# danieleschmidt/grid-fed-rl-gym

Measured on AMD Instinct MI355X. Metric: env steps/sec (batched feeders), higher is better.
Workload: dtype f64

## Files before the change

### grid_fed_rl_gym_amd/csrc/env_device.h

```cpp
#pragma once
#include <hip/hip_runtime.h>
#include <math.h>

#include "gs_internal.h"
#include "fastmath.h"

#ifndef ROW
#define ROW(r) S[(size_t)(r) * GS_LANES]
#endif

template <typename X>
__device__ __forceinline__ X cld(const X* p, int i) {
  return ((const GS_CONST X*)p)[i];
}

__device__ __forceinline__ double hour_of_day(double time_s) {
  return gs_fmod_pos(gs_div_by(time_s, 3600.0, 1.0 / 3600.0), 24.0, 1.0 / 24.0);
}

struct U4 { uint32_t a, b, c, d; };

__device__ __forceinline__ U4 philox(uint32_t c0, uint32_t c1, uint32_t c2, uint32_t c3, uint32_t k0, uint32_t k1) {
#pragma unroll
  for (int r = 0; r < 10; ++r) {
// ... 166 lines not shown
      ROW(R.SOC + q) = soc;
      ROW(R.BATP + q) = -(e * 3600.0 / dt);
    }
  }
#pragma unroll
  for (int g = 0; g < 8; ++g) { if (g >= T.n_gens) break; ROW(R.CURT + g) = (a_g[g] + 1.0) / 2.0; }
  for (int g = 8; g < T.n_gens; ++g) ROW(R.CURT + g) = (act[T.n_bats + g] + 1.0) / 2.0;
  ROW(R.TIME) = t_old + dt;
  ROW(R.STEP) = k_old + 1.0;
}

__device__ __forceinline__ double load_power_z(const GsTables& T, int l, double z, double prof) {
  return fmax(0.0, cld(T.load_base, l) * (prof * (1.0 + 0.1 * z)) * 1.0);
}
template <typename TablePtr>
__device__ __forceinline__ double daily_profile_from(TablePtr table, double time_s) {
  const double hour = hour_of_day(time_s);
  const int hi = (int)hour;
  const double frac = hour - (double)hi;
  return table[hi] * (1.0 - frac) + table[(hi + 1) % 24] * frac;
}
__device__ __forceinline__ double daily_profile(double time_s) { return daily_profile_from(kDailyProfile, time_s); }

__device__ __forceinline__ void bus_injection(const GsTables& T, const GsRows& R, const GsEnvCfg& E, GsLaneRows S, int i) {
  double ls = 0.0, gs = 0.0;
  for (int p = cld(T.bl_ptr, i); p < cld(T.bl_ptr, i + 1); ++p) ls += ROW(R.LOADP + cld(T.bl_idx, p));
  for (int p = cld(T.bg_ptr, i); p < cld(T.bg_ptr, i + 1); ++p) {
    const int g = cld(T.bg_idx, p);
    gs += ROW(R.GENP + g) * ROW(R.CURT + g);
  }
  for (int p = cld(T.bb_ptr, i); p < cld(T.bb_ptr, i + 1); ++p) {
    const double bp = ROW(R.BATP + cld(T.bb_idx, p));
    if (bp > 0.0) gs += bp; else if (bp < 0.0) ls += fabs(bp);
  }
  ROW(R.P + i) = (0.0 - gs_div_by(ls, E.power_base, E.inv_power_base)) + gs_div_by(gs, E.power_base, E.inv_power_base);
  ROW(R.Q + i) = 0.0;
}

__device__ __forceinline__ void env_reset_lane_scalars(const GsTables& T, const GsRows& R, const GsEnvCfg& E, GsLaneRows S,
                                                       uint64_t inst, uint64_t seed) {
  ROW(R.SEEDLO) = (double)(uint32_t)seed;
  ROW(R.SEEDHI) = (double)(uint32_t)(seed >> 32);
  ROW(R.TIME) = 0.0; ROW(R.STEP) = 0.0; ROW(R.VIOL) = 0.0; ROW(R.TOTLOSS) = 0.0; ROW(R.EPREW) = 0.0;
  ROW(R.FREQ) = 60.0;
  ROW(R.IRR) = 0.0; ROW(R.WIND) = 5.0; ROW(R.TEMP) = 25.0; ROW(R.CLOUD) = 0.3;
  for (int q = 0; q < T.n_bats; ++q) { ROW(R.SOC + q) = 0.5; ROW(R.BATP + q) = 0.0; }
// ... 25 lines not shown
```

### grid_fed_rl_gym_amd/csrc/gridstep_abi.hip

```cpp
#include <hip/hip_runtime.h>

#include <dlfcn.h>

#include <algorithm>
#include <cmath>
#include <cstdarg>
#include <cstdio>
#include <cstdlib>
#include <cstring>
#include <string>
#include <vector>

#include "../../include/gridstep.h"
#include "gs_internal.h"
#include "kernels.h"
#include "topology.h"
#include "mesh_schedule.h"
#include "plan.h"
#include "policy.h"

namespace {

thread_local std::string g_last_error;

// ... 33 lines not shown
  a.CommCuDevice = (int (*)(gs_ncclComm_t, int*))dlsym(lib, "ncclCommCuDevice");
  a.GetVersion = (int (*)(int*))dlsym(lib, "ncclGetVersion");
  a.GetErrorString = (const char* (*)(int))dlsym(lib, "ncclGetErrorString");
  if (!a.GetUniqueId || !a.CommInitRank || !a.AllGather || !a.CommDestroy) { why = "librccl lacks a required symbol"; return false; }
  g_rccl = a;
  return true;
}

struct TimedLaunch { int kid; hipEvent_t a, b; };
constexpr size_t GS_CHECKS_MAX_EVENTS = 4096;

}

struct gs_handle : GsPlan {
  int device = 0;
  hipStream_t stream = nullptr;
  gs_config cfg{};
  HostTopology topo;
  GsTables T{};
  struct gs_checks* fused = nullptr;
  bool forked = false;
  hipStream_t stream2 = nullptr; hipEvent_t ev_fork = nullptr, ev_join = nullptr, ev_peer = nullptr, ev_peer2 = nullptr;
  bool rows_stale = false; const double* last_obs = nullptr;
  unsigned long long* d_stamps = nullptr;
  bool was_reset = false;
  std::vector<void*> allocs;
  char* arena = nullptr; size_t arena_left = 0;
  double* slab = nullptr;
  double* d_in = nullptr; size_t in_doubles = 0;
  double* d_out = nullptr; size_t out_doubles = 0;
  double* d_obs2[2] = {nullptr, nullptr}; int obs_cur = 0;
  hipStream_t comm_stream = nullptr; hipEvent_t ev_step = nullptr, ev_gather[2] = {nullptr, nullptr}; bool gather_pending[2] = {false, false};
  std::vector<const double*> bound_obs;
  float* d_obs32 = nullptr;
  hipEvent_t ev_scalars = nullptr;
  double* d_actions = nullptr; int n_action_batches = 0;
  struct Rollout {
    int T_cap = 0, T = 0, term_cap = 0; uint64_t calls = 0;
    double* obs_seq = nullptr; double* act = nullptr; double* rew = nullptr; uint8_t* done = nullptr;
    int32_t* term_count = nullptr; int32_t* term_idx = nullptr; double* term_obs = nullptr;
    int32_t n_term = 0;
  } ro;
  struct Policy { bool set = false; double* blob = nullptr; double* act = nullptr; GsPolicyArgs args{}; int compute = GS_COMPUTE_F64; GsPolicyArgsF32 args32{}; int lds32 = 0; } pol;
  double* d_cst = nullptr;
  int32_t *map_obs = nullptr, *map_vm = nullptr, *map_va = nullptr, *map_flow = nullptr, *map_load = nullptr,
          *map_p = nullptr, *map_q = nullptr, *map_act = nullptr, *map_state = nullptr;
// ... 122 lines not shown
  HIPCHK(h, hipGetLastError());
  return GS_OK;
}

int launch_pack_obs(gs_handle* h, double* dst) {
  const int rc = launch_pack(h, h->map_obs, h->obs_dim, dst);
  if (rc || !h->pl) return rc;
  const size_t threads = (size_t)h->B * 2 * h->n_loads;
  hipLaunchKernelGGL(gs_k_load_columns, dim3((unsigned)((threads + 255) / 256)), dim3(256), 0, h->stream, (const double*)h->LL.pl, dst, h->B, h->obs_dim,
                     2 * h->n + 2 * h->m + 1, h->n_loads);
  HIPCHK(h, hipGetLastError());
  return GS_OK;
}

int launch_unpack(gs_handle* h, const int32_t* map, int C, const double* src, int stride = 0) {
  if (C <= 0) return GS_OK;
  LaunchTimer lt(h, GS_K_UNPACK);
  dim3 grid(h->groups, (C + 63) / 64);
  hipLaunchKernelGGL(gs_k_unpack, grid, dim3(256), 0, h->stream, map, C, h->R.total, h->slab, src, h->B, stride ? stride : C);
  HIPCHK(h, hipGetLastError());
  return GS_OK;
}

int ensure_rows(gs_handle* h) {
  if (!h->rows_stale) return GS_OK;
  h->rows_stale = false;
  return launch_unpack(h, h->map_obs, 2 * h->n + 2 * h->m, h->last_obs, h->obs_dim);
}

int pack_to_host(gs_handle* h, const int32_t* map, int C, double* host) {
  if (!host || C <= 0) return GS_OK;
  int rc = launch_pack(h, map, C, h->d_out);
  if (rc) return rc;
  HIPCHK(h, hipMemcpyAsync(host, h->d_out, (size_t)h->B * C * sizeof(double), hipMemcpyDeviceToHost, h->stream));
  HIPCHK(h, hipStreamSynchronize(h->stream));
  return GS_OK;
}

int unpack_from_host(gs_handle* h, const int32_t* map, int C, const double* host) {
  if (C <= 0) return GS_OK;
  HIPCHK(h, hipMemcpyAsync(h->d_in, host, (size_t)h->B * C * sizeof(double), hipMemcpyHostToDevice, h->stream));
  return launch_unpack(h, map, C, h->d_in);
}

int fetch_scalars(gs_handle* h, bool sync = true) {
  hipLaunchKernelGGL(gs_k_scalars, dim3(h->groups), dim3(64), 0, h->stream, h->rows_f, (int)SF_COUNT, h->rows_i,
                     (int)SI_COUNT, h->rows_u, (int)SU_COUNT, h->R.total, h->slab, h->hd_f, h->hd_i, h->hd_u, h->Bp, h->hd_v4, (int)SU_VF0);
// ... 31 lines not shown
  return GS_OK;
}

GsFusedChecks fused_checks_args(gs_handle* h);

int step_kernels(gs_handle* h, const double* d_actions, double* obs_out = nullptr, const GsRolloutStep* rs = nullptr) {
  { LaunchTimer lt(h, GS_K_SOLVE);
    dim3 grid(h->groups), block(64 * h->W);
    if (!obs_out) {
      const int next = h->obs_cur ^ 1;
      if (h->gather_pending[next]) {
        HIPCHK(h, hipStreamWaitEvent(h->stream, h->ev_gather[next], 0));
        if (h->split_ok) HIPCHK(h, hipStreamWaitEvent(h->stream2, h->ev_gather[next], 0));
        h->gather_pending[next] = false;
      }
      h->obs_cur = next;
      obs_out = h->d_obs2[next];
    }
    GsPackArgs pa{h->map_obs, h->d_cst, obs_out, h->obs_dim, (int)std::max<size_t>(1, std::min<size_t>(3, (h->dyn_lds - 49152) / (64 * 65 * sizeof(double)))), 0, 0,
                  h->obs_skip0, h->obs_skip1};
    pa.pair_ok = !(h->obs_dim & 1) && !((h->obs_skip1 - h->obs_skip0) & 1) && pa.tiles_per_pass >= 2 && !GS_EXPERIMENT_ENV("GS_PACK_BY_COLUMN");
    pa.early_pass0 = 2 * h->n + 2 * h->m >= 64 * pa.tiles_per_pass;
    pa.lean = h->lean ? 1 : 0;
    if (h->lean) { h->rows_stale = true; h->last_obs = obs_out; }
    const GsFusedChecks fc = fused_checks_args(h);
    const GsRolloutStep rsv = rs ? *rs : GsRolloutStep{};
    if (h->second_gen()) {
      const int per_group = 64 / h->f2().iw, n_wg = h->groups * per_group;
      const dim3 b2(64 * h->f2().nw);
      const bool split = h->split_ok && !h->timing;
      const int n_first = split ? (h->groups / 2) * per_group : n_wg;
      if (split && !h->forked) {
        HIPCHK(h, hipEventRecord(h->ev_fork, h->stream));
        HIPCHK(h, hipStreamWaitEvent(h->stream2, h->ev_fork, 0));
        h->forked = true;
      }
      GsF2Tables f2a = h->F2, f2b = h->F2;
      f2a.wg_offset = 0; f2b.wg_offset = n_first;
      auto launch = [&](auto k, auto... pz) -> int {
        if (!k) return fail(h, GS_E_STATE, "%s: no such step kernel", h->f2().name);
        hipLaunchKernelGGL(k, dim3(n_first), b2, h->F2.lds_bytes, h->stream, h->T, f2a, h->R, h->SC, h->EC, h->slab, h->B, d_actions, h->total_load, pa, fc, rsv, pz...);
        if (n_first < n_wg)
          hipLaunchKernelGGL(k, dim3(n_wg - n_first), b2, h->F2.lds_bytes, h->stream2, h->T, f2b, h->R, h->SC, h->EC, h->slab, h->B, d_actions, h->total_load, pa, fc, rsv, pz...);
        return GS_OK;
      };
      const GsStepKernels& k = gs_step_kernels[(int)h->step];
      const double *pz = h->LP.pz, *pl = h->LL.pl;
// ... 436 lines not shown
  if (mask) HIPCHK(h, hipMemcpyAsync(h->d_pzmask, mask, (size_t)h->B, hipMemcpyHostToDevice, h->stream));
  int rc = launch_line_params(h, mask ? h->d_pzmask : nullptr);
  if (rc) return rc;
  HIPCHK(h, hipStreamSynchronize(h->stream));
  return GS_OK;
}

int gs_get_line_impedances(const gs_handle* h, double* r, double* x) {
  if (!h) return fail(nullptr, GS_E_INVALID, "handle is NULL");
  if (!h->pz) return fail(const_cast<gs_handle*>(h), GS_E_STATE, "gs_get_line_impedances: the handle has no per-instance line impedances");
  if (r) std::copy(h->inst_r.begin(), h->inst_r.end(), r);
  if (x) std::copy(h->inst_x.begin(), h->inst_x.end(), x);
  return GS_OK;
}

int gs_set_load_powers(gs_handle* h, const double* base, const uint8_t* mask) {
  if (!h) return fail(nullptr, GS_E_INVALID, "handle is NULL");
  if (!h->pl) return fail(h, GS_E_STATE, "gs_set_load_powers: the handle was created without per-instance load powers "
                                         "(gs_topology::load_base_inst)");
  if (!base) return fail(h, GS_E_INVALID, "gs_set_load_powers: base is [B][n_loads]");
  const std::string why = gs_check_load_powers(h->n_loads, h->B, base, mask);
  if (!why.empty()) return fail(h, GS_E_INVALID, "%s", why.c_str());
  GS_ENTER(h);
  const size_t nl = (size_t)h->n_loads;
  for (int b = 0; b < h->B; ++b) {
    if (mask && !mask[b]) continue;
    std::copy(base + b * nl, base + (b + 1) * nl, h->inst_load.begin() + b * nl);
  }
  HIPCHK(h, hipMemcpyAsync(const_cast<double*>(h->LL.base), h->inst_load.data(), h->inst_load.size() * sizeof(double), hipMemcpyHostToDevice, h->stream));
  if (mask) HIPCHK(h, hipMemcpyAsync(h->d_plmask, mask, (size_t)h->B, hipMemcpyHostToDevice, h->stream));
  int rc = launch_load_params(h, mask ? h->d_plmask : nullptr);
  if (rc) return rc;
  HIPCHK(h, hipStreamSynchronize(h->stream));
  return GS_OK;
}

int gs_get_load_powers(const gs_handle* h, double* base) {
  if (!h) return fail(nullptr, GS_E_INVALID, "handle is NULL");
  if (!h->pl) return fail(const_cast<gs_handle*>(h), GS_E_STATE, "gs_get_load_powers: the handle has no per-instance load powers");
  if (base) std::copy(h->inst_load.begin(), h->inst_load.end(), base);
  return GS_OK;
}

static const char* const kPzNoSolve = "gs_solve / gs_solve_device: this handle has per-instance line impedances, which the solver API does not "
                                      "support (the step, rollout and fallback entry points do)";
int gs_upload_injections(gs_handle* h, const double* P_spec, const double* Q_spec) {
  if (!h || !P_spec) return fail(h, GS_E_INVALID, "handle / P_spec is NULL");
  if (h->pz) return fail(h, GS_E_STATE, "%s", kPzNoSolve);
  GS_ENTER(h);
  int rc = unpack_from_host(h, h->map_p, h->n, P_spec);
  if (rc) return rc;
  if (Q_spec) {
    HIPCHK(h, hipStreamSynchronize(h->stream));
    rc = unpack_from_host(h, h->map_q, h->n, Q_spec);
    if (rc) return rc;
  } else {
    hipLaunchKernelGGL(gs_k_fill_rows, dim3(h->groups), dim3(64), 0, h->stream, h->R.Q.base, 2, h->n, h->R.total, h->slab, 0.0);
    HIPCHK(h, hipGetLastError());
  }
  HIPCHK(h, hipStreamSynchronize(h->stream));
  return GS_OK;
}

int gs_solve_device(gs_handle* h) {
  if (!h) return fail(nullptr, GS_E_INVALID, "handle is NULL");
  if (h->pz) return fail(h, GS_E_STATE, "%s", kPzNoSolve);
  GS_ENTER(h);
  h->rows_stale = false;
  return launch_solve(h);
}

int gs_download_solution(gs_handle* h, const gs_solution_view* out) {
  if (!h || !out) return fail(h, GS_E_INVALID, "handle / view is NULL");
  GS_ENTER(h);
  int rc;
  if ((rc = ensure_rows(h))) return rc;
  if ((rc = pack_to_host(h, h->map_vm, h->n, out->bus_voltages))) return rc;
  if ((rc = pack_to_host(h, h->map_va, h->n, out->bus_angles))) return rc;
  if ((rc = pack_to_host(h, h->map_flow, h->m, out->line_flows))) return rc;
  if ((rc = pack_to_host(h, h->map_load, h->m, out->line_loadings))) return rc;
  if ((rc = fetch_scalars(h))) return rc;
  const int B = h->B, Bp = h->Bp;
  if (out->losses) memcpy(out->losses, h->h_f + (size_t)SF_LOSSES * Bp, B * sizeof(double));
  if (out->max_mismatch) memcpy(out->max_mismatch, h->h_f + (size_t)SF_MAXMIS * Bp, B * sizeof(double));
  if (out->iterations) memcpy(out->iterations, h->h_i + (size_t)SI_ITERS * Bp, B * sizeof(int32_t));
  if (out->status) memcpy(out->status, h->h_i + (size_t)SI_STATUS * Bp, B * sizeof(int32_t));
  if (out->converged) memcpy(out->converged, h->h_u + (size_t)SU_CONV * Bp, B);
  return GS_OK;
}

// ... 326 lines not shown
  gs_handle::Rollout& ro = h->ro;
  const size_t B = h->B, D = h->obs_dim, A = h->action_dim;
  ro.T = T; ro.n_term = -1;
  HIPCHK(h, hipMemsetAsync(ro.term_count, 0, sizeof(int32_t), h->stream));
  if (A > 0) {
    if (policy == GS_POLICY_UPLOADED) {
      HIPCHK(h, hipMemcpyAsync(ro.act, actions, (size_t)T * B * A * sizeof(double), hipMemcpyHostToDevice, h->stream));
    } else if (policy == GS_POLICY_RANDOM) {
      const long long total = (long long)T * B * ((A + 3) / 4);
      hipLaunchKernelGGL(gs_k_rollout_actions, dim3((unsigned)((total + 255) / 256)), dim3(256), 0, h->stream, ro.act, (int)T, (int)B, (int)A,
                         policy_seed, h->EC.first_instance, 0u);
      HIPCHK(h, hipGetLastError());
    }
  }
  HIPCHK(h, hipMemcpyAsync(ro.obs_seq, h->d_obs2[h->obs_cur], B * D * sizeof(double), hipMemcpyDeviceToDevice, h->stream));
  const bool fused = h->second_gen() && policy != GS_POLICY_MLP;
  for (int t = 0; t < T; ++t) {
    double* nxt = ro.obs_seq + (size_t)(t + 1) * B * D;
    if (policy == GS_POLICY_MLP && (rc = launch_policy(h, ro.obs_seq + (size_t)t * B * D, ro.act + (size_t)t * B * A, policy_seed, t))) return rc;
    GsRolloutStep rs{ro.rew, ro.done, ro.obs_seq + (size_t)t * B * D, h->map_obs, h->d_cst, ro.term_count, ro.term_idx, ro.term_obs, ro.term_cap, h->obs_dim, t, 1};
    if ((rc = step_kernels(h, ro.act + (size_t)t * B * A, nxt, fused ? &rs : nullptr))) return rc;
    if (!fused || t == T - 1) {
      if ((rc = join_streams(h))) return rc;
      GsRolloutPostArgs pa{fused ? nullptr : ro.rew, fused ? nullptr : ro.done, nxt, h->map_obs, h->d_cst, ro.term_count, ro.term_idx, ro.term_obs, ro.term_cap, h->obs_dim, t, h->B};
      hipLaunchKernelGGL(gs_k_rollout_post, dim3(h->groups), dim3(256), 0, h->stream, h->T, h->R, h->EC, h->slab, pa);
      HIPCHK(h, hipGetLastError());
      if (h->pl) {
        const size_t threads = (size_t)h->B * 2 * h->n_loads;
        hipLaunchKernelGGL(gs_k_load_columns, dim3((unsigned)((threads + 255) / 256)), dim3(256), 0, h->stream, (const double*)h->LL.pl, nxt, h->B,
                           h->obs_dim, 2 * h->n + 2 * h->m + 1, h->n_loads);
        HIPCHK(h, hipGetLastError());
      }
    }
  }
  if ((rc = join_streams(h))) return rc;
  if (h->gather_pending[h->obs_cur]) { HIPCHK(h, hipStreamWaitEvent(h->stream, h->ev_gather[h->obs_cur], 0)); h->gather_pending[h->obs_cur] = false; }
  HIPCHK(h, hipMemcpyAsync(h->d_obs2[h->obs_cur], ro.obs_seq + (size_t)T * B * D, B * D * sizeof(double), hipMemcpyDeviceToDevice, h->stream));
  if (h->rows_stale) h->last_obs = h->d_obs2[h->obs_cur];
  ro.calls += 1;
  return GS_OK;
}

static int rollout_finish(gs_handle* h) {
  gs_handle::Rollout& ro = h->ro;
  if (ro.T <= 0) return fail(h, GS_E_STATE, "no rollout has been collected on this handle");
  GS_ENTER(h);
  if (ro.n_term < 0) {
// ... 34 lines not shown
  if (ro.n_term && out->next_observations) {
    HIPCHK(h, hipMemcpyAsync(idx.data(), ro.term_idx, idx.size() * sizeof(int32_t), hipMemcpyDeviceToHost, h->stream));
    HIPCHK(h, hipMemcpyAsync(rows.data(), ro.term_obs, rows.size() * sizeof(double), hipMemcpyDeviceToHost, h->stream));
  }
  HIPCHK(h, hipStreamSynchronize(h->stream));
  if (out->next_observations)
    for (int k = 0; k < ro.n_term; ++k)
      memcpy(out->next_observations + ((size_t)idx[2 * k] * B + idx[2 * k + 1]) * D, rows.data() + (size_t)k * D, D * sizeof(double));
  if (out->n_terminal) *out->n_terminal = ro.n_term;
  return GS_OK;
}

int gs_get_state(gs_handle* h, double* state) {
  if (!h || !state) return fail(h, GS_E_INVALID, "handle / state is NULL");
  GS_ENTER(h);
  int rc = ensure_rows(h);
  if (rc) return rc;
  return pack_to_host(h, h->map_state, h->state_dim, state);
}

int gs_set_state(gs_handle* h, const double* state) {
  if (!h || !state) return fail(h, GS_E_INVALID, "handle / state is NULL");
  GS_ENTER(h);
  h->rows_stale = false;
  int rc = unpack_from_host(h, h->map_state, h->state_dim, state);
  if (rc) return rc;
  hipLaunchKernelGGL(gs_k_polar_to_rect, dim3(h->groups), dim3(64), 0, h->stream, h->T, h->R, h->slab, h->B);
  HIPCHK(h, hipGetLastError());
  if (h->comm_stream) HIPCHK(h, hipStreamSynchronize(h->comm_stream));
  h->gather_pending[0] = h->gather_pending[1] = false;
  if ((rc = launch_pack_obs(h, h->d_obs2[h->obs_cur]))) return rc;
  HIPCHK(h, hipMemcpyAsync(h->d_obs2[h->obs_cur ^ 1], h->d_obs2[h->obs_cur], (size_t)h->B * h->obs_dim * sizeof(double), hipMemcpyDeviceToDevice, h->stream));
  HIPCHK(h, hipStreamSynchronize(h->stream));
  h->was_reset = true;
  return GS_OK;
}

int gs_comm_unique_id(uint8_t id_out[128]) {
  std::string why;
  if (!load_rccl(why)) return fail(nullptr, GS_E_COMM, "%s", why.c_str());
  gs_ncclUniqueId id;
  int rc = g_rccl.GetUniqueId(&id);
  if (rc != 0) return fail(nullptr, GS_E_COMM, "ncclGetUniqueId: %s", g_rccl.GetErrorString ? g_rccl.GetErrorString(rc) : "error");
  memcpy(id_out, id.internal, 128);
  return GS_OK;
}
// ... 693 lines not shown
```

### grid_fed_rl_gym_amd/csrc/gs_internal.h

```cpp
#pragma once
#include <stdint.h>

#if defined(GS_BUILD_EXPERIMENTS)
#define GS_EXPERIMENT_ENV(name) getenv(name)
#else
#define GS_EXPERIMENT_ENV(name) ((const char*)nullptr)
#endif

#define GS_LANES 64
#define GS_ELEM(row, lane) ((((size_t)(row) >> 1) << 7) + ((size_t)(lane) << 1) + ((size_t)(row) & 1))
#define GS_MAX_WAVES 16
#define GS_ELL_K 4

#if defined(__HIP_DEVICE_COMPILE__)
#define GS_CONST __attribute__((address_space(4)))
#else
#define GS_CONST
#endif

#define GS_ARGS_IN_PLACE(Block, name)                                                                                           \
  const __attribute__((address_space(4))) char* ka_ = (const __attribute__((address_space(4))) char*)__builtin_amdgcn_kernarg_segment_ptr(); \
  asm volatile("" : "+s"(ka_));                                                                                                \
  const Block* name = (const Block*)ka_

// ... 312 lines not shown
  int32_t n_slots;
  int32_t slack;
  int32_t n_jump;
  int32_t n_levels, pos_off, n_anc_ints, wg_offset;
  int32_t off_tile, off_anc, off_z, off_env, off_red, off_atom, lds_bytes;
  int32_t off_prof, ring_zero;
  int32_t env_genp, env_curt, env_batp, env_soc;
  int32_t n_fixed, fixed_slot0;
  double fixed_val0;
  const int32_t* fixed_slot; const double* fixed_val;
  double* nrflat; int32_t nrflat_mode, pad_nrflat;
  const int32_t* mesh_items; const int32_t* mesh_rowinfo;
  int32_t off_scr, mesh_nz;
  int32_t mesh_pairs, mesh_off_p;
  const double* mesh_w; int32_t mesh_w_steps, mesh_slack;
};

struct GsRolloutPostArgs {
  double* rew; uint8_t* done;
  double* obs_next;
  const int32_t* map; const double* cst;
  int32_t* term_count; int32_t* term_idx; double* term_obs; int32_t term_cap;
  int32_t obs_dim, t, B;
};

struct GsRolloutStep {
  double* rew; uint8_t* done;
  double* obs_prev;
  const int32_t* map; const double* cst;
  int32_t* term_count; int32_t* term_idx; double* term_obs;
  int32_t term_cap, obs_dim, t, active;
};

#define GS_STAMP_BLOCKS 2048
struct GsSolveCfg {
  double tolerance, alpha;
  int32_t max_iterations, jacobian_exact;
  unsigned long long* stamps;
  int32_t stamp_wave, block_times;
};

struct GsEnvCfg {
  double timestep, v_min, v_max, f_min, f_max, safety_penalty, H, D, f0, power_base, inv_power_base;
  int32_t episode_length, stochastic_loads, weather_variation, fbs_warm_start;
  int64_t first_instance;
};
// ... 43 lines not shown
```

### grid_fed_rl_gym_amd/csrc/kernels.h

```cpp
#pragma once
#include <hip/hip_runtime.h>

#include <array>

#include "gs_internal.h"
#include "members.h"
#include "policy.h"

typedef void (*GsSolveFn)(GsTables T, GsRows R, GsSolveCfg C, double* slab, int B);
typedef void (*GsStepFn)(GsTables T, GsRows R, GsSolveCfg C, GsEnvCfg E, double* slab, int B, const double* actions, double total_load,
                         GsPackArgs PA, GsFusedChecks FC);
typedef void (*GsF2StepFn)(GsTables T, GsF2Tables F, GsRows R, GsSolveCfg C, GsEnvCfg E, double* slab, int B, const double* actions,
                           double total_load, GsPackArgs PA, GsFusedChecks FC, GsRolloutStep RS);
typedef void (*GsF2StepPzFn)(GsTables T, GsF2Tables F, GsRows R, GsSolveCfg C, GsEnvCfg E, double* slab, int B, const double* actions,
                             double total_load, GsPackArgs PA, GsFusedChecks FC, GsRolloutStep RS, const double* pz);
template <class Fn> struct GsStepFns { Fn step = nullptr, stepc = nullptr; };
struct GsSolveKernels { GsSolveFn solve; GsStepFns<GsStepFn> step; };
typedef void (*GsF2StepPzPlFn)(GsTables T, GsF2Tables F, GsRows R, GsSolveCfg C, GsEnvCfg E, double* slab, int B, const double* actions,
                               double total_load, GsPackArgs PA, GsFusedChecks FC, GsRolloutStep RS, const double* pz, const double* pl);
struct GsStepKernels { GsStepFns<GsF2StepFn> plain; GsStepFns<GsF2StepPzFn> pz, pl; GsStepFns<GsF2StepPzPlFn> pz_pl; };
extern const std::array<GsSolveKernels, (size_t)SolveMember::nr_sparse_lds + 1> gs_solve_kernels;
extern const std::array<GsStepKernels, kStepMemberCount> gs_step_kernels;

extern "C" {
__global__ void gs_k_line_params(GsLineParamArgs A);
__global__ void gs_k_load_params(GsLoadParamArgs A);
__global__ void gs_k_load_columns(const double* __restrict__ pl, double* __restrict__ out, int B, int obs_dim, int c0, int n_loads);
__global__ void gs_k_pre_nr_dmfma(GsTables T, GsRows R, GsSolveCfg C, GsEnvCfg E, double* __restrict__ slab, int B,
                                  const double* __restrict__ actions, double total_load, GsPackArgs PA, GsFusedChecks FC);
__global__ void gs_k_post_nr_dmfma(GsTables T, GsRows R, GsSolveCfg C, GsEnvCfg E, double* __restrict__ slab, int B,
                                   const double* __restrict__ actions, double total_load, GsPackArgs PA, GsFusedChecks FC);
__global__ void gs_k_postc_nr_dmfma(GsTables T, GsRows R, GsSolveCfg C, GsEnvCfg E, double* __restrict__ slab, int B,
                                    const double* __restrict__ actions, double total_load, GsPackArgs PA, GsFusedChecks FC);
__global__ void gs_k_posts_nr_dmfma(GsTables T, GsRows R, GsSolveCfg C, double* __restrict__ slab, int B);
__global__ void gs_k_nr_dense_mfma(GsDenseArgs A, double* __restrict__ slab, int B);
__global__ void gs_k_nr_dense_mfma2(GsDenseArgs A, double* __restrict__ slab, int B);
__global__ void gs_k_nr_sparse_lds(GsSparseArgs A, double* __restrict__ slab, int B);
__global__ void gs_k_env_reset(GsTables T, GsRows R, GsEnvCfg E, double* __restrict__ slab, int B,
                               const uint64_t* __restrict__ seeds, const uint8_t* __restrict__ mask);
__global__ void gs_k_polar_to_rect(GsTables T, GsRows R, double* __restrict__ slab, int B);
__global__ void gs_k_rollout_actions(double* __restrict__ act, int T, int B, int A, uint64_t seed, int64_t first_instance, uint32_t t0);
__global__ void gs_k_fill_const_columns(double* __restrict__ out, long long rows, int obs_dim, int skip0, int skip1,
                                        const int32_t* __restrict__ map, const double* __restrict__ cst);
__global__ void gs_k_policy_mlp(GsPolicyArgs P);
__global__ void gs_k_policy_mlp_f32(GsPolicyArgsF32 P);
__global__ void gs_k_rollout_post(GsTables T, GsRows R, GsEnvCfg E, double* __restrict__ slab, GsRolloutPostArgs A);
__global__ void gs_k_pack(const int32_t* __restrict__ src, const double* __restrict__ cst, int C, int rows_total,
                          const double* __restrict__ slab, double* __restrict__ out, int B);
__global__ void gs_k_unpack(const int32_t* __restrict__ dst, int C, int rows_total, double* __restrict__ slab,
                            const double* __restrict__ in, int B, int stride);
__global__ void gs_k_obs_compact(const double* __restrict__ src, double* __restrict__ dst, long long rows, int D, int skip0, int skip1, int expand);
__global__ void gs_k_obs_to_f32(const double* __restrict__ src, float* __restrict__ dst, long long n);
__global__ void gs_k_gather_lane(int row0, int count, int lane, const double* __restrict__ slab, double* __restrict__ out);
__global__ void gs_k_fill_rows(int row0, int stride, int count, int rows_total, double* __restrict__ slab, double value);
__global__ void gs_k_scalars(const int32_t* __restrict__ rf, int nf, const int32_t* __restrict__ ri, int ni,
                             const int32_t* __restrict__ ru, int nu, int rows_total, const double* __restrict__ slab,
                             double* __restrict__ of, int32_t* __restrict__ oi, uint8_t* __restrict__ ou, int Bp, uint32_t* __restrict__ ov4, int vf0);
__global__ void gs_k_checks(GsChecksCfg C, const double* __restrict__ slab, const double* __restrict__ freq_override,
                            double* __restrict__ prev, int32_t* __restrict__ state, int32_t* __restrict__ out_i,
                            double* __restrict__ out_f, uint8_t* __restrict__ bus_mask, uint8_t* __restrict__ line_mask, int B, int Bp);
__global__ void gs_k_fallback_linear(GsTables T, GsRows R, GsFallbackArgs A, double* __restrict__ slab, int B);
__global__ void gs_k_checks_reset(int32_t* __restrict__ state, const uint8_t* __restrict__ mask, int B, int Bp);
}
```

### grid_fed_rl_gym_amd/csrc/kernels_env.hip

```cpp
#include <hip/hip_runtime.h>
#include <math.h>

#include "gs_internal.h"

#define ROW(r) S[(size_t)(r) * GS_LANES]
#include "env_device.h"

extern "C" __global__ void __launch_bounds__(64)
gs_k_env_reset(GsTables T, GsRows R, GsEnvCfg E, double* __restrict__ slab, int B,
               const uint64_t* __restrict__ seeds, const uint8_t* __restrict__ mask) {
  const int lane = threadIdx.x;
  const int b = blockIdx.x * GS_LANES + lane;
  const GsLaneRows S = gs_lane_rows(slab, blockIdx.x, R.total, lane);
  if (b >= B) return;
  if (mask && !mask[b]) return;
  const uint64_t inst = (uint64_t)(E.first_instance + b);
  const uint64_t seed = seeds ? seeds[b] : next_episode_seed(lane_seed(S, R), inst);
  env_reset_lane(T, R, E, S, inst, seed);
}

extern "C" __global__ void __launch_bounds__(64)
gs_k_polar_to_rect(GsTables T, GsRows R, double* __restrict__ slab, int B) {
  const int lane = threadIdx.x;
  const int b = blockIdx.x * GS_LANES + lane;
  const GsLaneRows S = gs_lane_rows(slab, blockIdx.x, R.total, lane);
  if (b >= B) return;
  for (int i = 0; i < T.n; ++i) {
    const double vm = ROW(R.VM + i), va = ROW(R.VA + i);
    double s, c;
    sincos(va, &s, &c);
    ROW(R.E + i) = vm * c; ROW(R.F + i) = vm * s;
  }
  for (int g = 0; g < T.n_gens; ++g) ROW(R.GENP + g) = renewable_power(T, R, S, g);
}

extern "C" __global__ void __launch_bounds__(256)
gs_k_rollout_actions(double* __restrict__ act, int T, int B, int A, uint64_t seed, int64_t first_instance, uint32_t t0) {
  const int Aq = (A + 3) >> 2;
  const long long idx = (long long)blockIdx.x * blockDim.x + threadIdx.x;
  if (idx >= (long long)T * B * Aq) return;
  const int q = (int)(idx % Aq);
  const long long tb = idx / Aq;
  const int b = (int)(tb % B), t = (int)(tb / B);
  const U4 r = philox((uint32_t)(first_instance + b), t0 + (uint32_t)t, (uint32_t)q, 0x4143544Eu, (uint32_t)seed, (uint32_t)(seed >> 32));
  const uint32_t w[4] = {r.a, r.b, r.c, r.d};
  double* o = act + ((size_t)t * B + b) * A + 4 * q;
#pragma unroll
  for (int k = 0; k < 4; ++k)
    if (4 * q + k < A) o[k] = 2.0 * (((double)w[k] + 0.5) * (1.0 / 4294967296.0)) - 1.0;
}

extern "C" __global__ void __launch_bounds__(256)
gs_k_fill_const_columns(double* __restrict__ out, long long rows, int obs_dim, int skip0, int skip1,
                        const int32_t* __restrict__ map, const double* __restrict__ cst) {
  const int w = skip1 - skip0;
  const long long idx = (long long)blockIdx.x * blockDim.x + threadIdx.x;
// ... 18 lines not shown
        A.rew[(size_t)A.t * A.B + b] = rew;
        A.done[(size_t)A.t * A.B + b] = (uint8_t)d;
      }
      if (d) {
        k = atomicAdd(A.term_count, 1);
        if (k < A.term_cap) { A.term_idx[2 * k] = A.t; A.term_idx[2 * k + 1] = b; }
        else k = -1;
      }
    }
    fin[lane] = k;
  }
  __syncthreads();
  bool any = false;
  for (int q = 0; q < GS_LANES; ++q) {
    const int k = fin[q];
    any |= k != -2;
    if (k >= 0) {
      const double* row = A.obs_next + (size_t)(blockIdx.x * GS_LANES + q) * A.obs_dim;
      double* dst = A.term_obs + (size_t)k * A.obs_dim;
      for (int c = threadIdx.x; c < A.obs_dim; c += blockDim.x) dst[c] = row[c];
    }
  }
  if (!any) return;
  if (mine && fin[lane] != -2) {
    const uint64_t inst = (uint64_t)(E.first_instance + b);
    env_reset_lane_scalars(T, R, E, S, inst, next_episode_seed(lane_seed(S, R), inst));
  }
  for (int q = 0; q < GS_LANES; ++q) {
    if (fin[q] == -2) continue;
    const GsLaneRows Sq = gs_lane_rows(slab, blockIdx.x, R.total, q);
    for (int j = threadIdx.x; j < T.n + T.m; j += blockDim.x) env_reset_element(T, R, Sq, j);
  }
  asm volatile("s_waitcnt vmcnt(0) lgkmcnt(0)\n\ts_barrier" ::: "memory");
  for (int q = 0; q < GS_LANES; ++q) {
    if (fin[q] == -2) continue;
    const GsLaneRows Sq = gs_lane_rows(slab, blockIdx.x, R.total, q);
    double* row = A.obs_next + (size_t)(blockIdx.x * GS_LANES + q) * A.obs_dim;
    for (int c = threadIdx.x; c < A.obs_dim; c += blockDim.x) {
      const int s = A.map[c];
      row[c] = (s >= 0) ? Sq.lane_row((size_t)s * GS_LANES).get() : A.cst[-s - 1];
    }
  }
}
```

### grid_fed_rl_gym_amd/csrc/kernels_flow2.hip

```cpp
#include <hip/hip_runtime.h>
#include <math.h>
#include <limits.h>
#include <type_traits>
#include <utility>

#include "../../include/gridstep.h"
#include "gs_internal.h"
#include "kernels.h"
#include "members.h"

#define ROW(r) S[(size_t)(r) * GS_LANES]
#include "env_device.h"

#pragma clang fp contract(off)

extern __shared__ __attribute__((aligned(16))) char f2_lds[];

__device__ __forceinline__ void f2_sync() { asm volatile("s_waitcnt vmcnt(0) lgkmcnt(0)\n\ts_barrier" ::: "memory"); }
__device__ __forceinline__ void f2_lds_sync() { asm volatile("s_waitcnt lgkmcnt(0)\n\ts_barrier" ::: "memory"); }

#define F2_AS3 __attribute__((address_space(3)))
#define F2_P(type, off) ((type F2_AS3*)((F2_AS3 char*)f2_lds + (off)))
#define F2_VP(type, off) ((volatile type F2_AS3*)((F2_AS3 char*)f2_lds + (off)))
typedef double f2_v2 __attribute__((ext_vector_type(2)));
// ... 311 lines not shown
      if (on) { if (valid) f2_row(S, R.CURT + gi) = c; env_lds[(F.env_curt + gi) * IW + l] = c; }
    }
    if (valid && hv == 0) { ROW(R.TIME) = told + dt; ROW(R.STEP) = kold + 1.0; }
  }
  if (wave == (NW >= 2 ? 1 : 0)) {
    const GsWeather wx = weather_step(R, E, S, inst, tnew, snew, valid);
    const double elev = solar_elevation(valid ? tnew : told);
    for (int g0 = 0; g0 < ng; g0 += HV) {
      const int gi = g0 + hv; const bool on = gi < ng; const int gg = on ? gi : 0;
      const double cap = T.gen_cap[gg], p0 = T.gen_p0[gg], p1 = T.gen_p1[gg], p2 = T.gen_p2[gg];
      double pw;
      if (T.gen_kind[gg] == 0) {
        const double irr = 1000.0 * elev * (1.0 - 0.8 * wx.cloud);
        const double tf = 1.0 - 0.004 * fmax(0.0, wx.temp - 25.0);
        pw = fmin(irr * p1 * p0 * tf, cap);
      } else if (wx.wind < p0 || wx.wind > p2) pw = 0.0;
      else if (wx.wind <= p1) { const double q = (wx.wind - p0) / (p1 - p0); pw = cap * (q * q * q); }
      else pw = cap;
      if (on) { f2_row(S, R.GENP + gi) = pw; env_lds[(F.env_genp + gi) * IW + l] = pw; }
    }
  }
  if (NW < 3 || wave >= 2) {
    const double prof = E.stochastic_loads ? daily_profile_from(F2_P(const double, o_prof), tnew) : 1.0;
    for (int p = (NW < 3 ? wave : wave - 2) * HV + hv; 4 * p < nl_; p += (NW < 3 ? NW : NW - 2) * HV) {
      const int l0 = 4 * p;
      double base4[4];
#pragma unroll
      for (int k = 0; k < 4; ++k) base4[k] = PL ? 0.0 : T.load_base[min(l0 + k, nl_ - 1)];
      if constexpr (PL != 0) {
        const double2 b01 = pl_at(2 * p), b23 = pl_at(min(2 * p + 1, GS_PL_NP(nl_) - 1));
        base4[0] = b01.x; base4[1] = b01.y; base4[2] = b23.x; base4[3] = b23.y;
      }
      double z[4] = {0.0, 0.0, 0.0, 0.0};
      if (E.stochastic_loads) rng_normal_quad(seed, inst, snew, DRAW_LOAD0 + p, z);
      double lp[4];
#pragma unroll
      for (int k = 0; k < 4; ++k) {
        const double base = base4[k];
        lp[k] = E.stochastic_loads ? fmax(0.0, base * (prof * (1.0 + 0.1 * z[k])) * 1.0) : base;
        if (l0 + k < nl_) loadp_lds[(l0 + k) * IW + l] = lp[k];
      }
      if (l0 + 1 < nl_) f2_pair(S, R.LOADP + l0) = make_double2(lp[0], lp[1]); else f2_row(S, R.LOADP + l0) = lp[0];
      if (l0 + 3 < nl_) f2_pair(S, R.LOADP + l0 + 2) = make_double2(lp[2], lp[3]); else if (l0 + 2 < nl_) f2_row(S, R.LOADP + l0 + 2) = lp[2];
    }
  }
  stp.hit(F2_ST_PRO_SPARE);
  f2_lds_sync();
  stp.hit(F2_ST_PRO_SCALAR);

  double Pj[NI], IR[NI], II[NI], JR[NI], JI[NI];
#pragma unroll
  for (int j = 0; j < NI; ++j) {
    if constexpr (SOLVER == F2_NRM) { rdev[j][0] = *(const f2_i4*)&rec0[j].nl; rdev[j][1] = *(const f2_i4*)&rec0[j].g0; rdev_b1[j] = rec0[j].b1; }
    const int nl = rdev[j][0].x, l0 = rdev[j][0].y, l1 = rdev[j][0].z, ngj = rdev[j][0].w, g0 = rdev[j][1].x, g1 = rdev[j][1].y,
              nbj = rdev[j][1].z, b0 = rdev[j][1].w, b1 = rdev_b1[j];
    double ls = 0.0, gs = 0.0;
    if (nl > 0) ls += loadp_lds[l0 * IW + l];
    if (nl > 1) ls += loadp_lds[l1 * IW + l];
    if (ngj > 0) gs += env_lds[(F.env_genp + g0) * IW + l] * env_lds[(F.env_curt + g0) * IW + l];
    if (ngj > 1) gs += env_lds[(F.env_genp + g1) * IW + l] * env_lds[(F.env_curt + g1) * IW + l];
    if (nbj > 0) { const double bp = env_lds[(F.env_batp + b0) * IW + l]; if (bp > 0.0) gs += bp; else if (bp < 0.0) ls += fabs(bp); }
    if (nbj > 1) { const double bp = env_lds[(F.env_batp + b1) * IW + l]; if (bp > 0.0) gs += bp; else if (bp < 0.0) ls += fabs(bp); }
    Pj[j] = (0.0 - gs_div_by(ls, E.power_base, E.inv_power_base)) + gs_div_by(gs, E.power_base, E.inv_power_base);
    if constexpr (SOLVER == F2_NRM) {
      f2_st((unsigned)F.mesh_off_p + 64u * (unsigned)rec0[j].bus + ((unsigned)l << 3), Pj[j]);
    }
// ... 1295 lines not shown
```

Measured before the change: 261.5 million.

## Skip per-step LOADP slab writes in lean mode and recompute lazily on demand

In lean mode the fused flow kernel no longer writes per-lane load powers back to the global slab each step. A stale flag marks them invalid, and a new restore kernel (or the rollout post kernel on episode reset) recomputes them from the last step's time, step counter and RNG when anything needs them. This removes global memory stores from the hot step path. In exchange it adds recompute paths whose values must match bit-exactly, which is why the shared helpers use no-contract arithmetic.

```diff
diff --git a/grid_fed_rl_gym_amd/csrc/env_device.h b/grid_fed_rl_gym_amd/csrc/env_device.h
--- a/grid_fed_rl_gym_amd/csrc/env_device.h
+++ b/grid_fed_rl_gym_amd/csrc/env_device.h
@@ -212,6 +212,29 @@
 }
 __device__ __forceinline__ double daily_profile(double time_s) { return daily_profile_from(kDailyProfile, time_s); }
 
+template <int PL>
+__device__ __forceinline__ void load_base_quad(const GsTables& T, const double* pl_lane, int p, int nl, double (&base4)[4]) {
+  const int l0 = 4 * p;
+#pragma unroll
+  for (int k = 0; k < 4; ++k) base4[k] = PL ? 0.0 : T.load_base[min(l0 + k, nl - 1)];
+  if constexpr (PL != 0) {
+    const double2 b01 = *(const double2*)(pl_lane + (size_t)(2 * p) * (2 * GS_LANES));
+    const double2 b23 = *(const double2*)(pl_lane + (size_t)min(2 * p + 1, GS_PL_NP(nl) - 1) * (2 * GS_LANES));
+    base4[0] = b01.x; base4[1] = b01.y; base4[2] = b23.x; base4[3] = b23.y;
+  }
+}
+__device__ __forceinline__ void load_power_quad(const GsEnvCfg& E, uint64_t seed, uint64_t inst, uint32_t step, int p, double prof,
+                                                const double (&base4)[4], double (&lp)[4]) {
+  GS_NO_CONTRACT
+  double z[4] = {0.0, 0.0, 0.0, 0.0};
+  if (E.stochastic_loads) rng_normal_quad(seed, inst, step, DRAW_LOAD0 + p, z);
+#pragma unroll
+  for (int k = 0; k < 4; ++k) {
+    const double base = base4[k];
+    lp[k] = E.stochastic_loads ? fmax(0.0, base * (prof * (1.0 + 0.1 * z[k])) * 1.0) : base;
+  }
+}
+
 __device__ __forceinline__ void bus_injection(const GsTables& T, const GsRows& R, const GsEnvCfg& E, GsLaneRows S, int i) {
   double ls = 0.0, gs = 0.0;
   for (int p = cld(T.bl_ptr, i); p < cld(T.bl_ptr, i + 1); ++p) ls += ROW(R.LOADP + cld(T.bl_idx, p));
diff --git a/grid_fed_rl_gym_amd/csrc/gridstep_abi.hip b/grid_fed_rl_gym_amd/csrc/gridstep_abi.hip
--- a/grid_fed_rl_gym_amd/csrc/gridstep_abi.hip
+++ b/grid_fed_rl_gym_amd/csrc/gridstep_abi.hip
@@ -79,6 +79,7 @@
   bool forked = false;
   hipStream_t stream2 = nullptr; hipEvent_t ev_fork = nullptr, ev_join = nullptr, ev_peer = nullptr, ev_peer2 = nullptr;
   bool rows_stale = false; const double* last_obs = nullptr;
+  bool loadp_stale = false;
   unsigned long long* d_stamps = nullptr;
   bool was_reset = false;
   std::vector<void*> allocs;
@@ -247,7 +248,18 @@
   return GS_OK;
 }
 
+int ensure_loadp(gs_handle* h) {
+  if (!h->loadp_stale) return GS_OK;
+  h->loadp_stale = false;
+  LaunchTimer lt(h, GS_K_UNPACK);
+  hipLaunchKernelGGL(gs_k_restore_loadp, dim3(h->groups), dim3(256), 0, h->stream, h->T, h->R, h->EC, h->slab, h->B,
+                     h->pl ? (const double*)h->LL.pl : nullptr);
+  HIPCHK(h, hipGetLastError());
+  return GS_OK;
+}
+
 int ensure_rows(gs_handle* h) {
+  { const int rc = ensure_loadp(h); if (rc) return rc; }
   if (!h->rows_stale) return GS_OK;
   h->rows_stale = false;
   return launch_unpack(h, h->map_obs, 2 * h->n + 2 * h->m, h->last_obs, h->obs_dim);
@@ -325,7 +337,7 @@
     pa.pair_ok = !(h->obs_dim & 1) && !((h->obs_skip1 - h->obs_skip0) & 1) && pa.tiles_per_pass >= 2 && !GS_EXPERIMENT_ENV("GS_PACK_BY_COLUMN");
     pa.early_pass0 = 2 * h->n + 2 * h->m >= 64 * pa.tiles_per_pass;
     pa.lean = h->lean ? 1 : 0;
-    if (h->lean) { h->rows_stale = true; h->last_obs = obs_out; }
+    if (h->lean) { h->rows_stale = true; h->last_obs = obs_out; h->loadp_stale = true; }
     const GsFusedChecks fc = fused_checks_args(h);
     const GsRolloutStep rsv = rs ? *rs : GsRolloutStep{};
     if (h->second_gen()) {
@@ -808,6 +820,7 @@
   const std::string why = gs_check_load_powers(h->n_loads, h->B, base, mask);
   if (!why.empty()) return fail(h, GS_E_INVALID, "%s", why.c_str());
   GS_ENTER(h);
+  { int rc0 = ensure_loadp(h); if (rc0) return rc0; }
   const size_t nl = (size_t)h->n_loads;
   for (int b = 0; b < h->B; ++b) {
     if (mask && !mask[b]) continue;
@@ -852,6 +865,7 @@
   if (!h) return fail(nullptr, GS_E_INVALID, "handle is NULL");
   if (h->pz) return fail(h, GS_E_STATE, "%s", kPzNoSolve);
   GS_ENTER(h);
+  { int rc0 = ensure_loadp(h); if (rc0) return rc0; }
   h->rows_stale = false;
   return launch_solve(h);
 }
@@ -1224,7 +1238,8 @@
     if ((rc = step_kernels(h, ro.act + (size_t)t * B * A, nxt, fused ? &rs : nullptr))) return rc;
     if (!fused || t == T - 1) {
       if ((rc = join_streams(h))) return rc;
-      GsRolloutPostArgs pa{fused ? nullptr : ro.rew, fused ? nullptr : ro.done, nxt, h->map_obs, h->d_cst, ro.term_count, ro.term_idx, ro.term_obs, ro.term_cap, h->obs_dim, t, h->B};
+      GsRolloutPostArgs pa{fused ? nullptr : ro.rew, fused ? nullptr : ro.done, nxt, h->map_obs, h->d_cst, ro.term_count, ro.term_idx, ro.term_obs, ro.term_cap, h->obs_dim, t, h->B,
+                            h->loadp_stale ? 1 : 0, h->pl ? (const double*)h->LL.pl : nullptr};
       hipLaunchKernelGGL(gs_k_rollout_post, dim3(h->groups), dim3(256), 0, h->stream, h->T, h->R, h->EC, h->slab, pa);
       HIPCHK(h, hipGetLastError());
       if (h->pl) {
@@ -1305,6 +1320,7 @@
 int gs_set_state(gs_handle* h, const double* state) {
   if (!h || !state) return fail(h, GS_E_INVALID, "handle / state is NULL");
   GS_ENTER(h);
+  { int rc0 = ensure_loadp(h); if (rc0) return rc0; }
   h->rows_stale = false;
   int rc = unpack_from_host(h, h->map_state, h->state_dim, state);
   if (rc) return rc;
diff --git a/grid_fed_rl_gym_amd/csrc/gs_internal.h b/grid_fed_rl_gym_amd/csrc/gs_internal.h
--- a/grid_fed_rl_gym_amd/csrc/gs_internal.h
+++ b/grid_fed_rl_gym_amd/csrc/gs_internal.h
@@ -358,6 +358,8 @@
   const int32_t* map; const double* cst;
   int32_t* term_count; int32_t* term_idx; double* term_obs; int32_t term_cap;
   int32_t obs_dim, t, B;
+  int32_t lean;
+  const double* pl;
 };
 
 struct GsRolloutStep {
diff --git a/grid_fed_rl_gym_amd/csrc/kernels.h b/grid_fed_rl_gym_amd/csrc/kernels.h
--- a/grid_fed_rl_gym_amd/csrc/kernels.h
+++ b/grid_fed_rl_gym_amd/csrc/kernels.h
@@ -45,6 +45,7 @@
 __global__ void gs_k_policy_mlp(GsPolicyArgs P);
 __global__ void gs_k_policy_mlp_f32(GsPolicyArgsF32 P);
 __global__ void gs_k_rollout_post(GsTables T, GsRows R, GsEnvCfg E, double* __restrict__ slab, GsRolloutPostArgs A);
+__global__ void gs_k_restore_loadp(GsTables T, GsRows R, GsEnvCfg E, double* __restrict__ slab, int B, const double* __restrict__ pl);
 __global__ void gs_k_pack(const int32_t* __restrict__ src, const double* __restrict__ cst, int C, int rows_total,
                           const double* __restrict__ slab, double* __restrict__ out, int B);
 __global__ void gs_k_unpack(const int32_t* __restrict__ dst, int C, int rows_total, double* __restrict__ slab,
diff --git a/grid_fed_rl_gym_amd/csrc/kernels_env.hip b/grid_fed_rl_gym_amd/csrc/kernels_env.hip
--- a/grid_fed_rl_gym_amd/csrc/kernels_env.hip
+++ b/grid_fed_rl_gym_amd/csrc/kernels_env.hip
@@ -32,6 +32,36 @@
     ROW(R.E + i) = vm * c; ROW(R.F + i) = vm * s;
   }
   for (int g = 0; g < T.n_gens; ++g) ROW(R.GENP + g) = renewable_power(T, R, S, g);
+}
+
+template <int PL>
+__device__ __forceinline__ void loadp_rows_of_last_step(const GsTables& T, const GsRows& R, const GsEnvCfg& E, GsLaneRows S, int group, int lane,
+                                                        uint64_t inst, const double* __restrict__ pl, int p0, int dp) {
+  const int nl = T.n_loads;
+  const double tnew = ROW(R.TIME);
+  const uint32_t snew = (uint32_t)ROW(R.STEP);
+  const uint64_t seed = lane_seed(S, R);
+  const double* const pl_lane = PL ? pl + ((size_t)group * GS_PL_NQ(nl) * GS_LANES + lane) * 2 : nullptr;
+  const double prof = E.stochastic_loads ? daily_profile_from(kDailyProfile, tnew) : 1.0;
+  for (int p = p0; 4 * p < nl; p += dp) {
+    const int l0 = 4 * p;
+    double base4[4], lp[4];
+    load_base_quad<PL>(T, pl_lane, p, nl, base4);
+    load_power_quad(E, seed, inst, snew, p, prof, base4, lp);
+    if (l0 + 1 < nl) S.pair((size_t)(R.LOADP + l0) * GS_LANES) = make_double2(lp[0], lp[1]); else ROW(R.LOADP + l0) = lp[0];
+    if (l0 + 3 < nl) S.pair((size_t)(R.LOADP + l0 + 2) * GS_LANES) = make_double2(lp[2], lp[3]); else if (l0 + 2 < nl) ROW(R.LOADP + l0 + 2) = lp[2];
+  }
+}
+
+extern "C" __global__ void __launch_bounds__(256)
+gs_k_restore_loadp(GsTables T, GsRows R, GsEnvCfg E, double* __restrict__ slab, int B, const double* __restrict__ pl) {
+  const int lane = threadIdx.x & 63, wave = threadIdx.x >> 6;
+  const int b = blockIdx.x * GS_LANES + lane;
+  const GsLaneRows S = gs_lane_rows(slab, blockIdx.x, R.total, lane);
+  if (b >= B || (double)ROW(R.STEP) == 0.0) return;
+  const uint64_t inst = (uint64_t)(E.first_instance + b);
+  if (pl) loadp_rows_of_last_step<1>(T, R, E, S, blockIdx.x, lane, inst, pl, wave, 4);
+  else loadp_rows_of_last_step<0>(T, R, E, S, blockIdx.x, lane, inst, pl, wave, 4);
 }
 
 extern "C" __global__ void __launch_bounds__(256)
@@ -96,6 +126,14 @@
     }
   }
   if (!any) return;
+  if (A.lean) {
+    if (b < A.B && fin[lane] != -2) {
+      const uint64_t inst = (uint64_t)(E.first_instance + b);
+      if (A.pl) loadp_rows_of_last_step<1>(T, R, E, S, blockIdx.x, lane, inst, A.pl, threadIdx.x >> 6, 4);
+      else loadp_rows_of_last_step<0>(T, R, E, S, blockIdx.x, lane, inst, A.pl, threadIdx.x >> 6, 4);
+    }
+    __syncthreads();
+  }
   if (mine && fin[lane] != -2) {
     const uint64_t inst = (uint64_t)(E.first_instance + b);
     env_reset_lane_scalars(T, R, E, S, inst, next_episode_seed(lane_seed(S, R), inst));
diff --git a/grid_fed_rl_gym_amd/csrc/kernels_flow2.hip b/grid_fed_rl_gym_amd/csrc/kernels_flow2.hip
--- a/grid_fed_rl_gym_amd/csrc/kernels_flow2.hip
+++ b/grid_fed_rl_gym_amd/csrc/kernels_flow2.hip
@@ -357,26 +357,20 @@
   }
   if (NW < 3 || wave >= 2) {
     const double prof = E.stochastic_loads ? daily_profile_from(F2_P(const double, o_prof), tnew) : 1.0;
+    int loadp_row = PA.lean ? -1 : R.LOADP;
+    F2_OPAQUE(loadp_row);
     for (int p = (NW < 3 ? wave : wave - 2) * HV + hv; 4 * p < nl_; p += (NW < 3 ? NW : NW - 2) * HV) {
       const int l0 = 4 * p;
-      double base4[4];
-#pragma unroll
-      for (int k = 0; k < 4; ++k) base4[k] = PL ? 0.0 : T.load_base[min(l0 + k, nl_ - 1)];
-      if constexpr (PL != 0) {
-        const double2 b01 = pl_at(2 * p), b23 = pl_at(min(2 * p + 1, GS_PL_NP(nl_) - 1));
-        base4[0] = b01.x; base4[1] = b01.y; base4[2] = b23.x; base4[3] = b23.y;
-      }
-      double z[4] = {0.0, 0.0, 0.0, 0.0};
-      if (E.stochastic_loads) rng_normal_quad(seed, inst, snew, DRAW_LOAD0 + p, z);
-      double lp[4];
-#pragma unroll
-      for (int k = 0; k < 4; ++k) {
-        const double base = base4[k];
-        lp[k] = E.stochastic_loads ? fmax(0.0, base * (prof * (1.0 + 0.1 * z[k])) * 1.0) : base;
+      double base4[4], lp[4];
+      load_base_quad<PL>(T, pl_lane, p, nl_, base4);
+      load_power_quad(E, seed, inst, snew, p, prof, base4, lp);
+#pragma unroll
+      for (int k = 0; k < 4; ++k)
         if (l0 + k < nl_) loadp_lds[(l0 + k) * IW + l] = lp[k];
-      }
-      if (l0 + 1 < nl_) f2_pair(S, R.LOADP + l0) = make_double2(lp[0], lp[1]); else f2_row(S, R.LOADP + l0) = lp[0];
-      if (l0 + 3 < nl_) f2_pair(S, R.LOADP + l0 + 2) = make_double2(lp[2], lp[3]); else if (l0 + 2 < nl_) f2_row(S, R.LOADP + l0 + 2) = lp[2];
+      if (__builtin_amdgcn_readfirstlane(loadp_row) >= 0) {
+        if (l0 + 1 < nl_) f2_pair(S, loadp_row + l0) = make_double2(lp[0], lp[1]); else f2_row(S, loadp_row + l0) = lp[0];
+        if (l0 + 3 < nl_) f2_pair(S, loadp_row + l0 + 2) = make_double2(lp[2], lp[3]); else if (l0 + 2 < nl_) f2_row(S, loadp_row + l0 + 2) = lp[2];
+      }
     }
   }
   stp.hit(F2_ST_PRO_SPARE);
```

Measured after the change: 261.5 million. No clear change (-0.0%).
